# Hi-PACE/hipace

Measured on AMD Instinct MI355X. Metric: transverse slices/s at 1024^2 x 4ppc (explicit solver), higher is better.
Workload: dtype f64

## Files before the change

hipace_amd/csrc/particles_tiled.hip:

```cpp
#include "common.h"
#include <type_traits>
#include "particle_math.h"
#include "tiling.h"
#include "mg_gate.h"
#include "beam_deposit.h"

#include <algorithm>
#include <atomic>
#include <cstdio>
#include <cstdlib>
#include <cstring>
#include <mutex>
#include <set>
#include <string>

namespace hps {

static std::atomic<bool> g_record{false};
static std::mutex g_record_mu;
static std::set<std::string> g_recorded;
static void record_launch (const char* kernel, std::initializer_list<int> args)
{
    std::string n(kernel);
    char sep = '<';
    for (int a : args) { char b[16]; std::snprintf(b, sizeof b, "%c%d", sep, a); n += b; sep = ','; }
    n += '>';
    std::lock_guard<std::mutex> lk(g_record_mu);
    g_recorded.insert(n);
}
#define HPS_RECORD(kernel, ...) do { if (__builtin_expect(g_record.load(std::memory_order_relaxed), 0)) record_launch(kernel, {__VA_ARGS__}); } while (0)

static int expl_pad ()
{
    static int pad = -1;
    if (pad < 0) {
        pad = 2;
        if (const char* e = std::getenv("HPS_EXPL_PAD")) { const int v = std::atoi(e); if (v == 2 || v == 8) pad = v; }
    }
    return pad;
}
constexpr int TILE_HALO = 6;

#ifdef HPS_STAMPS
__device__ long long* g_pt_dbg = nullptr;
#define PT_STAMP(i) do { if (g_pt_dbg && blockIdx.x == 2000 && threadIdx.x == 0) g_pt_dbg[i] = __builtin_amdgcn_s_memtime(); } while (0)
#else
#define PT_STAMP(i) do { } while (0)
#endif

struct CompSlots { int n; int comp[6]; };

typedef __attribute__((address_space(3))) double lds_double;

__device__ __forceinline__ void lds_add (double* p, double v)
{
    __hip_atomic_fetch_add((lds_double*)p, v, __ATOMIC_RELAXED, __HIP_MEMORY_SCOPE_WORKGROUP);
}
__device__ __forceinline__ double lds_get (const double* p)
{
    return *(const lds_double*)p;
}

template <int ORDER>
__device__ __forceinline__ double laser_gather_lds (const double* a, int pitch, int li, int lj, const double* lx, const double* ly)
{
    double A = 0.0;
#pragma unroll
    for (int iy = 0; iy <= ORDER; ++iy)
#pragma unroll
        for (int ix = 0; ix <= ORDER; ++ix) A += lx[ix]*ly[iy]*lds_get(a + (lj + iy)*pitch + li + ix);
    return A;
}
template <int ORDER>
__device__ __forceinline__ void laser_gather_grad_lds (const double* a, int pitch, int li, int lj, const double* lx, const double* ly,
                                                       double dx_inv, double dy_inv, double& A, double& ADx, double& ADy)
{
    A = 0.0; ADx = 0.0; ADy = 0.0;
#pragma unroll
    for (int iy = 0; iy <= ORDER; ++iy)
#pragma unroll
        for (int ix = 0; ix <= ORDER; ++ix) {
            const double* c = a + (lj + iy)*pitch + li + ix;
            const double w = lx[ix]*ly[iy];
            A += w*lds_get(c);
            ADx += w*0.5*dx_inv*(lds_get(c + 1) - lds_get(c - 1));
            ADy += w*0.5*dy_inv*(lds_get(c + pitch) - lds_get(c - pitch));
        }
}

__device__ __forceinline__ int4 tile_record (const int* __restrict__ offsets, const TailWork& tw, long n, bool& tail)
{
    const int b0 = (int)blockIdx.x - tw.extra;
    const int b = b0 - tw.nwg;
    tail = b < 0;
    if (tail) {
        const long nn = tw.live_n ? (long)*tw.live_n : n;
        const long first = (long)tw.first + 256L*b0;
        return make_int4(0, (int)min(first, nn), (int)min(first + 256, nn), 0);
    }
    return reinterpret_cast<const int4*>(offsets + tile_launch_offset(gridDim.x - tw.nwg - tw.extra))[b];
}
constexpr int TAIL_ORIGIN = -(1 << 24);

template <int R, int RP = R, int NT = 256, int NC = 6>
__device__ __forceinline__ void load_region (double* img, const SlabView& f, const int* comps, int nc, int ox, int oy, int tid);

template <int ORDER, int TS, int MASK, bool LASER = false, bool VBW = false>
__global__ __launch_bounds__(256)
void k_deposit_tiled (SlabView f, hps_plasma pl, const int* __restrict__ offsets, int ntx, DepComps cm,
                      PartConsts k, int* n_qsa, int* n_fallback, const int* __restrict__ tile_flag, TailWork tw, BeamPairWork bw,
                      const int* go)
{
    if (go && *go == 0) return;
    if ((int)blockIdx.x < bw.nwg) {
        beam_pair_block<ORDER>(f, bw, (int)blockIdx.x, k.dx_inv, k.dy_inv, k.xoff, k.yoff);
        return;
    }
    constexpr int R = TS + 2*TILE_HALO;
    constexpr int RP = R, PL = RP*R;
    if (tile_flag && !tile_flag[offsets[gridDim.x + 2 + blockIdx.x]]) return;
    extern __shared__ __attribute__((aligned(16))) double acc[];
    const int gc[6] = {cm.jx, cm.jy, cm.jz, cm.rho, cm.chi, cm.rhomjz};
    int slot[6]; int na = 0;
#pragma unroll
    for (int c = 0; c < 6; ++c) {
        const bool on = (MASK >= 0) ? ((MASK >> c) & 1) : (gc[c] >= 0);
        slot[c] = on ? na++ : -1;
    }

    bool tail;
    const int4 lrec = tile_record(offsets, tw, pl.n, tail);
    const int tile = lrec.x;
    const int ox = tail ? TAIL_ORIGIN : (tile % ntx)*TS - TILE_HALO, oy = tail ? TAIL_ORIGIN : (tile / ntx)*TS - TILE_HALO;
    const int tid = threadIdx.x;
    PT_STAMP(0);
    const int pend = lrec.z;
    int nfb = 0;
    struct Rec { double x, y, w, ux, uy, psi; uint64_t id; int ion; };
    auto fetch = [&] (int ip) {
        Rec r;
        r.x = pl.x[ip]; r.y = pl.y[ip]; r.w = pl.w[ip];
        r.ux = pl.ux[ip]; r.uy = pl.uy[ip]; r.psi = pl.psi[ip];
        if constexpr (VBW) r.id = (r.w != 0.0) ? HPS_ID_VALID : 0ULL;
        else r.id = pl.idcpu[ip];
        r.ion = k.can_ionize ? pl.ion_lev[ip] : 1;
        return r;
    };
    constexpr int NB = 4;
    Rec rec[NB];
    const int ipb = lrec.y + tid;
    if (ipb < pend) {
#pragma unroll
        for (int u = 0; u < NB; ++u) rec[u] = fetch(min(ipb + 256*u, pend - 1));
    }
    {
        double2* z = (double2*)acc;
        for (int s = tid; s < na*PL/2; s += 256) z[s] = make_double2(0.0, 0.0);
    }
    double* aimg = acc + na*PL;
    if constexpr (LASER) { const int ca[1] = {k.aabs}; load_region<R, R, 256, 1>(aimg, f, ca, 1, ox, oy, tid); }
    __syncthreads();
    PT_STAMP(1);

    for (int ip0 = ipb; ip0 < pend; ip0 += 256*NB) {
      if (ip0 != ipb) {
#pragma unroll
        for (int u = 0; u < NB; ++u) rec[u] = fetch(min(ip0 + 256*u, pend - 1));
      }
#pragma unroll
      for (int u = 0; u < NB; ++u) {
        const int ip = ip0 + 256*u;
        if (ip >= pend) break;
        const Rec cur = rec[u];
        const uint64_t id = cur.id;
        if (!(id & HPS_ID_VALID)) continue;
        const double psi_inv = 1.0/cur.psi;
        const double vx_c = cur.ux*psi_inv;
        const double vy_c = cur.uy*psi_inv;
        double q_invvol = k.a*cur.w;
        double q_mu0_mass = k.b;
        if (k.can_ionize) { const double il = (double)cur.ion; q_invvol *= il; q_mu0_mass *= il; }
        double sx[ORDER + 1], sy[ORDER + 1];
        const int i0 = shape_weights<ORDER>((cur.x - k.xoff)*k.dx_inv, sx);
        const int j0 = shape_weights<ORDER>((cur.y - k.yoff)*k.dy_inv, sy);
        const int li = i0 - ox, lj = j0 - oy;
        const bool local = (li >= 0 && li + ORDER < R && lj >= 0 && lj + ORDER < R);
        double gamma_psi;
        if constexpr (LASER) {
            double A = (local ? laser_gather_lds<ORDER>(aimg, R, li, lj, sx, sy)
                              : laser_gather<ORDER>(f, k.aabs, (cur.x - k.xoff)*k.dx_inv, (cur.y - k.yoff)*k.dy_inv))*k.laser_fac;
            if (k.can_ionize) A *= (double)cur.ion*(double)cur.ion;
            gamma_psi = 0.5*((1.0 + 0.5*A)*psi_inv*psi_inv + vx_c*vx_c*k.c_inv*k.c_inv + vy_c*vy_c*k.c_inv*k.c_inv + 1.0);
        } else {
            gamma_psi = 0.5*(psi_inv*psi_inv + vx_c*vx_c*k.c_inv*k.c_inv + vy_c*vy_c*k.c_inv*k.c_inv + 1.0);
        }
        if (gamma_psi < 0.0 || gamma_psi > k.max_qsa || psi_inv < 0.0) {
            if (n_qsa) atomicAdd(n_qsa, 1);
            pl.w[ip] = 0.0;
            pl.idcpu[ip] = (VBW ? pl.idcpu[ip] : id) & ~HPS_ID_VALID;
            if (pl.psi_half) pl.psi_half[ip] = 0.0;
            continue;
        }
        if (k.can_ionize && cur.ion == 0) continue;
        const double wv[6] = {vx_c, vy_c, (gamma_psi - 1.0)*k.c, gamma_psi, q_mu0_mass*psi_inv, 1.0};
        if (local) {
#pragma unroll
            for (int iy = 0; iy <= ORDER; ++iy) {
#pragma unroll
                for (int ix = 0; ix <= ORDER; ++ix) {
                    const double cd = q_invvol*sx[ix]*sy[iy];
                    double* p = acc + (lj + iy)*RP + li + ix;
#pragma unroll
                    for (int c = 0; c < 6; ++c) if (slot[c] >= 0) lds_add(p + slot[c]*PL, cd*wv[c]);
                }
            }
        } else {
            nfb += !tail;
#pragma unroll
            for (int iy = 0; iy <= ORDER; ++iy) {
#pragma unroll
                for (int ix = 0; ix <= ORDER; ++ix) {
                    const double cd = q_invvol*sx[ix]*sy[iy];
                    double* p = f.p + f.off(i0 + ix, j0 + iy);
#pragma unroll
                    for (int c = 0; c < 6; ++c) if (slot[c] >= 0) atomic_add_f64(p + gc[c]*f.ns, cd*wv[c]);
                }
            }
        }
      }
    }
    if (n_fallback && nfb) atomicAdd(n_fallback, nfb);
    PT_STAMP(2);
    __syncthreads();
    PT_STAMP(3);

    for (int s = tid; s < R*R; s += 256) {
        const int lj = s / R, li = s - lj*R;
        const int i = ox + li, j = oy + lj;
        if (i < -f.ng || i >= f.nx + f.ng || j < -f.ng || j >= f.ny + f.ng) continue;
        double* p = f.p + f.off(i, j);
#pragma unroll
        for (int c = 0; c < 6; ++c) {
            if (slot[c] >= 0) {
                const double v = acc[slot[c]*PL + lj*RP + li];
                if (v != 0.0) atomic_add_f64(p + gc[c]*f.ns, v);
            }
        }
    }
    PT_STAMP(4);
}

template <int R, int RP, int NT, int NC>
__device__ __forceinline__ void load_region (double* img, const SlabView& f, const int* comps, int nc, int ox, int oy, int tid)
{
    constexpr int NIT = (R*R + NT - 1)/NT;
    double v[NIT][NC];
#pragma unroll
    for (int it = 0; it < NIT; ++it) {
        const int s = min(tid + it*NT, R*R - 1);
        const int lj = s / R, li = s - lj*R;
        const int i = ox + li, j = oy + lj;
        const bool in = (i >= -f.ng && i < f.nx + f.ng && j >= -f.ng && j < f.ny + f.ng);
        const long o = in ? f.off(i, j) : 0;
#pragma unroll
        for (int c = 0; c < NC; ++c) { v[it][c] = 0.0; if (c < nc) { const double q = f.p[comps[c]*f.ns + o]; v[it][c] = in ? q : 0.0; } }
    }
#pragma unroll
    for (int it = 0; it < NIT; ++it) {
        const int s = tid + it*NT;
        if (s < R*R) {
            const int lj = s / R, li = s - lj*R;
#pragma unroll
            for (int c = 0; c < NC; ++c) if (c < nc) img[c*RP*R + lj*RP + li] = v[it][c];
        }
    }
}

template <int ORDER, int DT, int TS, bool LASER = false, int PAD = 2, bool VBW = false>
__global__ __launch_bounds__(256) __attribute__((amdgpu_waves_per_eu(4, 4)))
void k_explicit_tiled (SlabView f, hps_plasma pl, const int* __restrict__ offsets, int ntx,
                       int cBz, int cEz, int cExmBy, int cEypBx, int cSy, int cSx, PartConsts k, int* n_fallback,
                       const int* __restrict__ tile_flag, TailWork tw)
{
    constexpr int R = TS + 2*TILE_HALO;
    constexpr int RP = R + PAD, PL = RP*R;
    if (tile_flag && !tile_flag[offsets[gridDim.x + 2 + blockIdx.x]]) return;
    constexpr int NS = ORDER + DT + 1;
    extern __shared__ __attribute__((aligned(16))) double lds[];
    double* img = lds;
    double* acc = lds + 4*PL;
    double* aimg = lds + 6*PL;
    bool tail;
    const int4 lrec = tile_record(offsets, tw, pl.n, tail);
    const int tile = lrec.x;
    const int ox = tail ? TAIL_ORIGIN : (tile % ntx)*TS - TILE_HALO, oy = tail ? TAIL_ORIGIN : (tile / ntx)*TS - TILE_HALO;
    const int tid = threadIdx.x;
    const int cc[4] = {cBz, cEz, cExmBy, cEypBx};
    const int pend = lrec.z;
    struct Rec { double x, y, w, ux, uy, psi; uint64_t id; int ion; };
    auto fetch = [&] (int ip) {
        Rec r;
        r.x = pl.x[ip]; r.y = pl.y[ip]; r.w = pl.w[ip];
        r.ux = pl.ux[ip]; r.uy = pl.uy[ip]; r.psi = pl.psi[ip];
        if constexpr (VBW) r.id = (r.w != 0.0) ? HPS_ID_VALID : 0ULL;
        else r.id = pl.idcpu[ip];
        r.ion = k.can_ionize ? pl.ion_lev[ip] : 1;
        return r;
    };
    const int ipb = lrec.y + tid;
    Rec nxt{};
    if (ipb < pend) nxt = fetch(ipb);
    load_region<R, RP, 256, 4>(img, f, cc, 4, ox, oy, tid);
    if constexpr (LASER) { const int ca[1] = {k.aabs}; load_region<R, RP, 256, 1>(aimg, f, ca, 1, ox, oy, tid); }
    {
        double2* z = (double2*)acc;
        for (int s = tid; s < PL; s += 256) z[s] = make_double2(0.0, 0.0);
    }
    __syncthreads();

    int nfb = 0;
    bool slow = false;
    auto one = [&] (const Rec& cur, auto LC) __attribute__((always_inline)) -> bool {
        constexpr bool LOCAL = decltype(LC)::value;
        if (!(cur.id & HPS_ID_VALID)) return true;
        if (k.can_ionize && cur.ion == 0) return true;
        const double xmid = (cur.x - k.xoff)*k.dx_inv;
        const double ymid = (cur.y - k.yoff)*k.dy_inv;
        double sx[NS], dsx[NS], sy[NS], dsy[NS];
        int i0, j0;
        if constexpr (DT == 2) { i0 = centred_weights<ORDER>(xmid, sx, dsx); j0 = centred_weights<ORDER>(ymid, sy, dsy); }
        else                   { i0 = nodal_weights<ORDER>(xmid, sx, dsx);   j0 = nodal_weights<ORDER>(ymid, sy, dsy); }
        const int li = i0 - ox, lj = j0 - oy;
        const bool local = LASER ? (li >= 1 && li + NS + 1 <= R && lj >= 1 && lj + NS + 1 <= R)
                                 : (li >= 0 && li + NS <= R && lj >= 0 && lj + NS <= R);
        if (local != LOCAL) return false;
        const double psi_inv = fast_rcp(cur.psi);
        const double vx = cur.ux*psi_inv*k.c_inv;
        const double vy = cur.uy*psi_inv*k.c_inv;
        double q_invvol_mu0 = k.a, q_mass = k.b;
        if (k.can_ionize) { const double il = (double)cur.ion; q_invvol_mu0 *= il; q_mass *= il; }
        const double cdm = q_invvol_mu0*cur.w;
        double gp;
        if constexpr (LASER) {
            double lx[ORDER + 1], ly[ORDER + 1];
            const int ai = shape_weights<ORDER>(xmid, lx), aj = shape_weights<ORDER>(ymid, ly);
            const double A = (LOCAL ? laser_gather_lds<ORDER>(aimg, RP, ai - ox, aj - oy, lx, ly)
                                    : laser_gather<ORDER>(f, k.aabs, xmid, ymid))*k.laser_fac*q_mass*q_mass;
            gp = 0.5*((1.0 + 0.5*A)*psi_inv*psi_inv + vx*vx + vy*vy + 1.0);
        } else {
            gp = 0.5*(psi_inv*psi_inv + vx*vx + vy*vy + 1.0);
        }
        const double qp = q_mass*psi_inv;
        const double vxvy = vx*vy, gy = gp - vy*vy, gx = gp - vx*vx;
        const double cq = cdm*qp, cqc = cq*k.c_inv, cc = cdm*k.c;
        const double a1 = cq*vx, a2 = -cqc*vy, a3 = cqc*vxvy, a4 = -cqc*gy, a5 = cc*vxvy, a6 = -cc*(gy - 1.0);
        const double b1 = cq*vy, b2 = cqc*vx, b3 = cqc*gx, b4 = -cqc*vxvy, b5 = cc*(gx - 1.0), b6 = -cc*vxvy;
#pragma unroll
        for (int m = 0; m < NS; ++m) { dsx[m] *= k.dx_inv; dsy[m] *= k.dy_inv; }
#pragma unroll
        for (int iy = 0; iy < NS; ++iy) {
            if constexpr (LOCAL) asm volatile("" ::: "memory");
            const bool yedge = (DT == 2) && (iy == 0 || iy == NS - 1);
            const double a5s = a5*sy[iy], b5s = b5*sy[iy], ay = a6*dsy[iy], by = b6*dsy[iy];
#pragma unroll
            for (int ix = 0; ix < NS; ++ix) {
                const bool xedge = (DT == 2) && (ix == 0 || ix == NS - 1);
                if (xedge && yedge) continue;
                double* gp_ = nullptr; int ls = 0;
                if constexpr (LOCAL) ls = (lj + iy)*RP + li + ix;
                else                 gp_ = f.p + f.off(i0 + ix, j0 + iy);
                double sy_add, sx_add;
                if (xedge)      { sy_add = a5s*dsx[ix]; sx_add = b5s*dsx[ix]; }
                else if (yedge) { sy_add = ay*sx[ix];   sx_add = by*sx[ix]; }
                else {
                    double Bz, Ez, ExmBy, EypBx;
                    if constexpr (LOCAL) { Bz = lds_get(img + ls); Ez = lds_get(img + PL + ls); ExmBy = lds_get(img + 2*PL + ls); EypBx = lds_get(img + 3*PL + ls); }
                    else                 { Bz = gp_[cBz*f.ns]; Ez = gp_[cEz*f.ns]; ExmBy = gp_[cExmBy*f.ns]; EypBx = gp_[cEypBx*f.ns]; }
                    double ty = fma(a1, Bz, fma(a2, Ez, fma(a3, ExmBy, a4*EypBx)));
                    double tx = fma(b1, Bz, fma(b2, Ez, fma(b3, ExmBy, b4*EypBx)));
                    if constexpr (LASER) {
                        if (sx[ix]*sy[iy] != 0.0) {
                            const double lf = 0.25*cq*qp*k.laser_fac*k.c;
                            double ady, adx;
                            if constexpr (LOCAL) {
                                const double* a = aimg + ls;
                                ady = lds_get(a + RP) - lds_get(a - RP); adx = lds_get(a + 1) - lds_get(a - 1);
                            } else {
                                const double* a = f.p + k.aabs*f.ns + f.off(i0 + ix, j0 + iy);
                                ady = a[f.js] - a[-f.js]; adx = a[1] - a[-1];
                            }
                            ty = fma(lf*0.5*k.dy_inv, ady, ty);
                            tx = fma(-lf*0.5*k.dx_inv, adx, tx);
                        }
                    }
                    sy_add = fma(sx[ix], fma(sy[iy], ty, ay), a5s*dsx[ix]);
                    sx_add = fma(sx[ix], fma(sy[iy], tx, by), b5s*dsx[ix]);
                }
                if constexpr (LOCAL) { lds_add(acc + ls, sy_add); lds_add(acc + PL + ls, sx_add); }
                else                 { atomic_add_f64(gp_ + cSy*f.ns, sy_add); atomic_add_f64(gp_ + cSx*f.ns, sx_add); }
            }
        }
        return true;
    };
    for (int ip = ipb; ip < pend; ip += 256) {
        const Rec cur = nxt;
        if (ip + 256 < pend) nxt = fetch(ip + 256);
        if (!one(cur, std::true_type{})) { slow = true; nfb += !tail; }
    }
    if (slow) {
#pragma unroll 1
        for (int ip = ipb; ip < pend; ip += 256) { const Rec cur = fetch(ip); (void)one(cur, std::false_type{}); }
    }
    if (n_fallback && nfb) atomicAdd(n_fallback, nfb);
    __syncthreads();
#ifdef HPS_DIAG_EXPL_NO_FLUSH
    if (acc[tid] == 1.2345e-300 && n_fallback) atomicAdd(n_fallback, 1);
    return;
#endif
    for (int s = tid; s < R*R; s += 256) {
        const int lj = s / R, li = s - lj*R;
        const int i = ox + li, j = oy + lj;
        if (i < -f.ng || i >= f.nx + f.ng || j < -f.ng || j >= f.ny + f.ng) continue;
        double* p = f.p + f.off(i, j);
        const double a = acc[lj*RP + li], b = acc[PL + lj*RP + li];
        if (a != 0.0) atomic_add_f64(p + cSy*f.ns, a);
        if (b != 0.0) atomic_add_f64(p + cSx*f.ns, b);
    }
}

template <class T> __device__ __forceinline__ T ldo (const T* base, unsigned o) { return *reinterpret_cast<const T*>(reinterpret_cast<const char*>(base) + o); }
template <class T> __device__ __forceinline__ void sto (T* base, unsigned o, T v) { *reinterpret_cast<T*>(reinterpret_cast<char*>(base) + o) = v; }
template <class T> __device__ __forceinline__ T ldo_nt (const T* base, unsigned o) { return __builtin_nontemporal_load(reinterpret_cast<const T*>(reinterpret_cast<const char*>(base) + o)); }
template <class T> __device__ __forceinline__ void sto_nt (T* base, unsigned o, T v) { __builtin_nontemporal_store(v, reinterpret_cast<T*>(reinterpret_cast<char*>(base) + o)); }

struct DepTail { DepComps cm; double a, b, max_qsa; int* n_qsa; };
template <int ORDER, int TS, bool LASER = false, bool IONIZE = false, bool VBP = false, int DEP = 0>
__global__ __launch_bounds__(256) __attribute__((amdgpu_waves_per_eu(IONIZE ? 2 : 3)))
void k_advance_tiled (SlabView f, hps_plasma pl, const int* __restrict__ offsets, int ntx,
                      int cPsi, int cEz, int cBx, int cBy, int cBz, PartConsts k, int* n_fallback, IonArgs ia, const int* go, TailWork tw, MgPost mp,
                      DepTail dt)
{
    static_assert(DEP == 0 || (!LASER && !IONIZE), "the deposition tail exists for the plain push only");
    constexpr int R = TS + 2*TILE_HALO;
    constexpr int NS = ORDER + 2;
    static_assert(!(VBP && IONIZE), "the ADK draw is keyed by the id");
    int go_now;
    if (mp.src) {
        go_now = vcycle_active(mp.after) ? 0 : 1;
        if (blockIdx.x == 0) {
            for (int w = threadIdx.x; w < mp.nwords; w += 256) mp.dst[w] = mp.src[w];
            HPS_HOST_STORES_ACKNOWLEDGED();
            __syncthreads();
            if (threadIdx.x == 0) *mp.seq_slot = mp.seq;
        }
    } else go_now = go ? *go : 1;
    int charged = 0;
    extern __shared__ __attribute__((aligned(16))) double img[];
    bool tail;
    const int4 lrec = tile_record(offsets, tw, pl.n, tail);
    const int tile = lrec.x;
    if constexpr (IONIZE) {
        if (!go_now) return;
        if (ia.fbound && ia.tile_flag && ia.tile_flag[tile] == 0 && adk_tile_below_threshold(ia, tile % ntx, tile / ntx)) {
            adk_post(ia);
            return;
        }
    }
    const int ox = tail ? TAIL_ORIGIN : (tile % ntx)*TS - TILE_HALO, oy = tail ? TAIL_ORIGIN : (tile / ntx)*TS - TILE_HALO;
    const int tid = threadIdx.x;
    const unsigned pend = (unsigned)lrec.z;
    struct PIn { uint64_t id; double xp, yp, uxh, uyh, psih; };
    auto fetch = [&] (unsigned ip) {
        PIn q;
        const unsigned o = ip*8u;
        if constexpr (!VBP) q.id = ldo(pl.idcpu, o);
        q.xp = ldo(pl.x_prev, o); q.yp = ldo(pl.y_prev, o);
        q.uxh = ldo_nt(pl.ux_half, o); q.uyh = ldo_nt(pl.uy_half, o); q.psih = ldo_nt(pl.psi_half, o);
        if constexpr (VBP) q.id = (q.psih != 0.0) ? HPS_ID_VALID : 0ULL;
        return q;
    };
    unsigned ip = (unsigned)lrec.y + tid;
    PIn nxt{0, 0.0, 0.0, 0.0, 0.0, 1.0};
    if (ip < pend) nxt = fetch(ip);
    const int cc[5] = {cPsi, cEz, cBx, cBy, cBz};
    load_region<R, R, 256, 5>(img, f, cc, 5, ox, oy, tid);
    double* aimg = img + 5*R*R;
    if constexpr (LASER) { const int ca[1] = {k.aabs}; load_region<R, R, 256, 1>(aimg, f, ca, 1, ox, oy, tid); }
    __syncthreads();
    if (!go_now) return;
    int nfb = 0;

    for (; ip < pend; ip += 256) {
        __builtin_assume(ip < (1u << 28));
        const PIn cur = nxt;
        if (ip + 256 < pend) nxt = fetch(ip + 256);
        const unsigned o8 = ip*8u;
        const uint64_t id = cur.id;
        if (!(id & HPS_ID_VALID)) continue;
        double qmc = k.a;
        if (k.can_ionize) qmc *= (double)pl.ion_lev[ip];
        bool dead = false;
        for (int isc = 0; isc < k.n_subcycles && !dead; ++isc) {
            double xp = isc == 0 ? cur.xp : ldo(pl.x_prev, o8);
            double yp = isc == 0 ? cur.yp : ldo(pl.y_prev, o8);
            double sx[NS], dsx[NS], sy[NS], dsy[NS];
            constexpr bool W3 = ORDER == 2;
            double pxw[3] = {0.0, 0.0, 0.0}, pyw[3] = {0.0, 0.0, 0.0}; bool xhw = false, yhw = false;
            int i0, j0;
            if constexpr (W3) {
                i0 = nodal_weights2_w3((xp - k.xoff)*k.dx_inv, sx, dsx, pxw, xhw);
                j0 = nodal_weights2_w3((yp - k.yoff)*k.dy_inv, sy, dsy, pyw, yhw);
            } else {
                i0 = nodal_weights<ORDER>((xp - k.xoff)*k.dx_inv, sx, dsx);
                j0 = nodal_weights<ORDER>((yp - k.yoff)*k.dy_inv, sy, dsy);
            }
            const int li = i0 - ox, lj = j0 - oy;
            const bool local = (li >= 0 && li + NS <= R && lj >= 0 && lj + NS <= R);
            if (!local && !tail) ++nfb;
            Fld F{0, 0, 0, 0, 0, 0};
            if (local) {
                const double* b = img + lj*R + li;
#pragma unroll
                for (int iy = 0; iy < NS; ++iy) {
                    double rp = 0.0, rd = 0.0;
#pragma unroll
                    for (int ix = 0; ix < NS; ++ix) {
                        const double psi_c = lds_get(b + iy*R + ix);
                        rp = fma(sx[ix], psi_c, rp);
                        rd = fma(dsx[ix], psi_c, rd);
                    }
                    F.ExmBy = fma(sy[iy], rd, F.ExmBy);
                    F.EypBx = fma(dsy[iy], rp, F.EypBx);
                }
                const bool xhi = W3 ? xhw : !(sx[NS - 1] == 0.0), yhi = W3 ? yhw : !(sy[NS - 1] == 0.0);
                double px[NS - 1], py[NS - 1];
#pragma unroll
                for (int m = 0; m < NS - 1; ++m) {
                    if constexpr (W3) { px[m] = pxw[m < 3 ? m : 2]; py[m] = pyw[m < 3 ? m : 2]; }
                    else { px[m] = xhi ? sx[m + 1] : sx[m]; py[m] = yhi ? sy[m + 1] : sy[m]; }
                }
                const double* bq = b + R*R + (yhi ? R : 0) + (xhi ? 1 : 0);
#pragma unroll
                for (int ky = 0; ky < NS - 1; ++ky) {
                    asm volatile("" ::: "memory");
                    double rez = 0.0, rbx = 0.0, rby = 0.0, rbz = 0.0;
#pragma unroll
                    for (int kx = 0; kx < NS - 1; ++kx) {
                        const int ls = ky*R + kx;
                        rez = fma(px[kx], lds_get(bq + ls), rez);
                        rbx = fma(px[kx], lds_get(bq + R*R + ls), rbx);
                        rby = fma(px[kx], lds_get(bq + 2*R*R + ls), rby);
                        rbz = fma(px[kx], lds_get(bq + 3*R*R + ls), rbz);
                    }
                    F.Ez  = fma(py[ky], rez, F.Ez);
                    F.Bxc = fma(py[ky], rbx, F.Bxc);
                    F.Byc = fma(py[ky], rby, F.Byc);
                    F.Bz  = fma(py[ky], rbz, F.Bz);
                }
                F.ExmBy *= k.dx_inv;
                F.EypBx *= k.dy_inv;
            } else {
#ifdef HPS_DIAG_PUSH_NO_FALLBACK
                F.Ez = 1.0;
#else
#pragma unroll 1
                for (int iy = 0; iy < NS; ++iy) {
#pragma unroll
                    for (int ix = 0; ix < NS; ++ix) {
                        const double* p = f.p + f.off(i0 + ix, j0 + iy);
                        const double psi_c = p[cPsi*f.ns];
                        const double ss = sx[ix]*sy[iy];
                        F.ExmBy += (dsx[ix]*sy[iy])*psi_c*k.dx_inv;
                        F.EypBx += (sx[ix]*dsy[iy])*psi_c*k.dy_inv;
                        F.Ez  += ss*p[cEz*f.ns];
                        F.Bxc += ss*p[cBx*f.ns];
                        F.Byc += ss*p[cBy*f.ns];
                        F.Bz  += ss*p[cBz*f.ns];
                    }
                }
#endif
            }
            F.Bxc *= k.c;
            F.Byc *= k.c;
            if constexpr (IONIZE) {
                if (isc == 0) {
                    int lev = pl.ion_lev[ip];
                    const double uxh = cur.uxh, uyh = cur.uyh;
                    const bool ionize = lev < ia.Z && adk_decide(ia, F.ExmBy + F.Byc, F.EypBx - F.Bxc, F.Ez, uxh, uyh, cur.psih, lev, id);
                    if (ionize) { ++lev; pl.ion_lev[ip] = lev; qmc = k.a*(double)lev; }
                    adk_emit(ia, ionize, pl.x[ip], pl.y[ip], xp, yp, pl.w[ip]);
                    charged |= (lev > 0);
                    if (lev == 0 && uxh == 0.0 && uyh == 0.0) break;
                }
            }
            LaserFld Lf{0.0, 0.0, 0.0};
            if constexpr (LASER) {
                double lx[ORDER + 1], ly[ORDER + 1];
                const int ai = shape_weights<ORDER>((xp - k.xoff)*k.dx_inv, lx) - ox, aj = shape_weights<ORDER>((yp - k.yoff)*k.dy_inv, ly) - oy;
                if (ai >= 1 && ai + ORDER + 1 < R && aj >= 1 && aj + ORDER + 1 < R)
                    laser_gather_grad_lds<ORDER>(aimg, R, ai, aj, lx, ly, k.dx_inv, k.dy_inv, Lf.A, Lf.ADx, Lf.ADy);
                else
                    laser_gather_grad<ORDER>(f, k.aabs, (xp - k.xoff)*k.dx_inv, (yp - k.yoff)*k.dy_inv, k.dx_inv, k.dy_inv, Lf.A, Lf.ADx, Lf.ADy);
                const double ln = k.laser_fac*(k.can_ionize ? (double)pl.ion_lev[ip]*(double)pl.ion_lev[ip] : 1.0);
                Lf.A *= 0.5*ln; Lf.ADx *= 0.25*k.c*ln; Lf.ADy *= 0.25*k.c*ln;
            }
            const double dz = k.dz, sdz = dz*0.25;
            double ux = isc == 0 ? cur.uxh : ldo(pl.ux_half, o8), uy = isc == 0 ? cur.uyh : ldo(pl.uy_half, o8), psi = isc == 0 ? cur.psih : ldo(pl.psi_half, o8);
            const PushForce PFc = push_force(F, Lf, k.c_inv, qmc);
            const double h2 = 0.5*sdz*sdz;
#pragma unroll 1
            for (int s = 0; s < 4; ++s) taylor2_substep_pre<LASER>(ux, uy, psi, PFc, sdz, h2);
            const double pinv = fast_rcp(psi);
            xp += dz*k.c_inv*(ux*pinv);
            yp += dz*k.c_inv*(uy*pinv);
            if (apply_particle_bc(k, xp, yp, ux, uy)) {
                sto(pl.w, o8, 0.0);
                sto(pl.idcpu, o8, (uint64_t)((VBP ? ldo(pl.idcpu, o8) : id) & ~HPS_ID_VALID));
                sto(pl.psi_half, o8, 0.0);
                dead = true;
                break;
            }
            sto(pl.x, o8, xp); sto(pl.y, o8, yp);
            if (!k.temp_slice) {
                sto_nt(pl.ux_half, o8, ux); sto_nt(pl.uy_half, o8, uy); sto_nt(pl.psi_half, o8, psi);
                if (pl.x_prev != pl.x) sto(pl.x_prev, o8, xp);
                if (pl.y_prev != pl.y) sto(pl.y_prev, o8, yp);
            }
#pragma unroll 1
            for (int s = 0; s < 2; ++s) taylor2_substep_pre<LASER>(ux, uy, psi, PFc, sdz, h2);
            sto(pl.ux, o8, ux); sto(pl.uy, o8, uy); sto(pl.psi, o8, psi);
        }
    }
    if constexpr (DEP != 0) {
        constexpr int RR = R*R;
        const int gc[6] = {dt.cm.jx, dt.cm.jy, dt.cm.jz, dt.cm.rho, dt.cm.chi, dt.cm.rhomjz};
        int slot[6]; int na = 0;
#pragma unroll
        for (int c = 0; c < 6; ++c) { const bool on = (DEP >> c) & 1; slot[c] = on ? na++ : -1; }
        __syncthreads();
        double* acc = img;
        {   double2* z = (double2*)acc;
            for (int s2 = tid; s2 < na*RR/2; s2 += 256) z[s2] = make_double2(0.0, 0.0); }
        __syncthreads();
        for (unsigned iq = (unsigned)lrec.y + tid; iq < pend; iq += 256) {
            const unsigned o = iq*8u;
            auto ldc2 = [] (const double* base, unsigned off) {
                return __hip_atomic_load(reinterpret_cast<const double*>(reinterpret_cast<const char*>(base) + off), __ATOMIC_RELAXED, __HIP_MEMORY_SCOPE_AGENT); };
            const double w = ldc2(pl.w, o);
            const double x = ldc2(pl.x, o), y = ldc2(pl.y, o), ux = ldc2(pl.ux, o), uy = ldc2(pl.uy, o), psi = ldc2(pl.psi, o);
            if (w == 0.0) continue;
            const double psi_inv = 1.0/psi;
            const double vx_c = ux*psi_inv, vy_c = uy*psi_inv;
            const double q_invvol = dt.a*w;
            const double gamma_psi = 0.5*(psi_inv*psi_inv + vx_c*vx_c*k.c_inv*k.c_inv + vy_c*vy_c*k.c_inv*k.c_inv + 1.0);
            if (gamma_psi < 0.0 || gamma_psi > dt.max_qsa || psi_inv < 0.0) {
                if (dt.n_qsa) atomicAdd(dt.n_qsa, 1);
                sto(pl.w, o, 0.0);
                sto(pl.idcpu, o, (uint64_t)(ldo(pl.idcpu, o) & ~HPS_ID_VALID));
                sto(pl.psi_half, o, 0.0);
                continue;
            }
            double wx[ORDER + 1], wy[ORDER + 1];
            const int i0 = shape_weights<ORDER>((x - k.xoff)*k.dx_inv, wx);
            const int j0 = shape_weights<ORDER>((y - k.yoff)*k.dy_inv, wy);
            const double wv[6] = {vx_c, vy_c, (gamma_psi - 1.0)*k.c, gamma_psi, dt.b*psi_inv, 1.0};
            const int li = i0 - ox, lj = j0 - oy;
            if (li >= 0 && li + ORDER < R && lj >= 0 && lj + ORDER < R) {
#pragma unroll
                for (int iy = 0; iy <= ORDER; ++iy) {
#pragma unroll
                    for (int ix = 0; ix <= ORDER; ++ix) {
                        const double cd = q_invvol*wx[ix]*wy[iy];
                        double* p = acc + (lj + iy)*R + li + ix;
#pragma unroll
                        for (int c = 0; c < 6; ++c) if (slot[c] >= 0) lds_add(p + slot[c]*RR, cd*wv[c]);
                    }
                }
            } else {
                nfb += !tail;
#pragma unroll
                for (int iy = 0; iy <= ORDER; ++iy) {
#pragma unroll
                    for (int ix = 0; ix <= ORDER; ++ix) {
                        const double cd = q_invvol*wx[ix]*wy[iy];
                        double* p = f.p + f.off(i0 + ix, j0 + iy);
#pragma unroll
                        for (int c = 0; c < 6; ++c) if (slot[c] >= 0) atomic_add_f64(p + gc[c]*f.ns, cd*wv[c]);
                    }
                }
            }
        }
        __syncthreads();
        for (int s2 = tid; s2 < RR; s2 += 256) {
            const int lj = s2 / R, li = s2 - lj*R;
            const int i = ox + li, j = oy + lj;
            if (i < -f.ng || i >= f.nx + f.ng || j < -f.ng || j >= f.ny + f.ng) continue;
            double* p = f.p + f.off(i, j);
#pragma unroll
            for (int c = 0; c < 6; ++c) {
                if (slot[c] >= 0) {
                    const double v = acc[slot[c]*RR + s2];
                    if (v != 0.0) atomic_add_f64(p + gc[c]*f.ns, v);
                }
            }
        }
    }
    if (n_fallback && nfb) atomicAdd(n_fallback, nfb);
    if constexpr (IONIZE) {
        const int any = __syncthreads_or(charged);
        if (ia.tile_flag && tid == 0) ia.tile_flag[tile] = any;
        adk_post(ia);
    }
}

template <int ORDER, int TS, int MASK, int NT>
__global__ __launch_bounds__(NT)
void k_advance_deposit_tiled (SlabView f, hps_plasma pl, const int* __restrict__ offsets, int ntx,
                              int cPsi, int cEz, int cBx, int cBy, int cBz, PartConsts k, DepComps cm, PartConsts kd,
                              int* n_qsa, int* n_fallback)
{
    constexpr int R = TS + 2*TILE_HALO;
    constexpr int NS = ORDER + 2;
    extern __shared__ __attribute__((aligned(16))) double img[];
    double* acc = img + 5*R*R;
    const int gc[6] = {cm.jx, cm.jy, cm.jz, cm.rho, cm.chi, cm.rhomjz};
    int slot[6]; int na = 0;
#pragma unroll
    for (int c = 0; c < 6; ++c) { const bool on = (MASK >> c) & 1; slot[c] = on ? na++ : -1; }
    const int tile = offsets[gridDim.x + 2 + blockIdx.x];
    const int ox = (tile % ntx)*TS - TILE_HALO, oy = (tile / ntx)*TS - TILE_HALO;
    const int tid = threadIdx.x;
    const int cc[5] = {cPsi, cEz, cBx, cBy, cBz};
    load_region<R, R, NT, 5>(img, f, cc, 5, ox, oy, tid);
    {
        double2* z = (double2*)acc;
        for (int s = tid; s < na*R*R/2; s += NT) z[s] = make_double2(0.0, 0.0);
    }
    __syncthreads();

    const int pend = offsets[tile + 1];
    int nfb = 0;
    for (int ip = offsets[tile] + tid; ip < pend; ip += NT) {
        const uint64_t id = pl.idcpu[ip];
        if (!(id & HPS_ID_VALID)) continue;
        const double qmc = k.a;
        bool dead = false;
        double xp = 0.0, yp = 0.0, ux = 0.0, uy = 0.0, psi = 1.0;
        for (int isc = 0; isc < k.n_subcycles && !dead; ++isc) {
            xp = pl.x_prev[ip];
            yp = pl.y_prev[ip];
            double sx[NS], dsx[NS], sy[NS], dsy[NS];
            const int i0 = nodal_weights<ORDER>((xp - k.xoff)*k.dx_inv, sx, dsx);
            const int j0 = nodal_weights<ORDER>((yp - k.yoff)*k.dy_inv, sy, dsy);
            const int li = i0 - ox, lj = j0 - oy;
            const bool local = (li >= 0 && li + NS <= R && lj >= 0 && lj + NS <= R);
            if (!local) ++nfb;
            Fld F{0, 0, 0, 0, 0, 0};
            if (local) {
                const double* b = img + lj*R + li;
#pragma unroll 1
                for (int iy = 0; iy < NS; ++iy) {
                    double rp = 0.0, rd = 0.0, rez = 0.0, rbx = 0.0, rby = 0.0, rbz = 0.0;
#pragma unroll
                    for (int ix = 0; ix < NS; ++ix) {
                        const int ls = iy*R + ix;
                        const double psi_c = lds_get(b + ls);
                        rp = fma(sx[ix], psi_c, rp);
                        rd = fma(dsx[ix], psi_c, rd);
                        rez = fma(sx[ix], lds_get(b + R*R + ls), rez);
                        rbx = fma(sx[ix], lds_get(b + 2*R*R + ls), rbx);
                        rby = fma(sx[ix], lds_get(b + 3*R*R + ls), rby);
                        rbz = fma(sx[ix], lds_get(b + 4*R*R + ls), rbz);
                    }
                    F.ExmBy = fma(sy[iy], rd, F.ExmBy);
                    F.EypBx = fma(dsy[iy], rp, F.EypBx);
                    F.Ez  = fma(sy[iy], rez, F.Ez);
                    F.Bxc = fma(sy[iy], rbx, F.Bxc);
                    F.Byc = fma(sy[iy], rby, F.Byc);
                    F.Bz  = fma(sy[iy], rbz, F.Bz);
                }
                F.ExmBy *= k.dx_inv;
                F.EypBx *= k.dy_inv;
            } else {
#pragma unroll 1
                for (int iy = 0; iy < NS; ++iy) {
#pragma unroll
                    for (int ix = 0; ix < NS; ++ix) {
                        const double* p = f.p + f.off(i0 + ix, j0 + iy);
                        const double psi_c = p[cPsi*f.ns];
                        const double ss = sx[ix]*sy[iy];
                        F.ExmBy += (dsx[ix]*sy[iy])*psi_c*k.dx_inv;
                        F.EypBx += (sx[ix]*dsy[iy])*psi_c*k.dy_inv;
                        F.Ez  += ss*p[cEz*f.ns];
                        F.Bxc += ss*p[cBx*f.ns];
                        F.Byc += ss*p[cBy*f.ns];
                        F.Bz  += ss*p[cBz*f.ns];
                    }
                }
            }
            F.Bxc *= k.c;
            F.Byc *= k.c;
            const double dz = k.dz, sdz = dz*0.25;
            ux = pl.ux_half[ip]; uy = pl.uy_half[ip]; psi = pl.psi_half[ip];
#pragma unroll 1
            for (int s = 0; s < 4; ++s) taylor2_substep(ux, uy, psi, F, k.c_inv, qmc, sdz);
            const double pinv = fast_rcp(psi);
            xp += dz*k.c_inv*(ux*pinv);
            yp += dz*k.c_inv*(uy*pinv);
            if (apply_particle_bc(k, xp, yp, ux, uy)) {
                pl.w[ip] = 0.0;
                pl.idcpu[ip] = id & ~HPS_ID_VALID;
                pl.psi_half[ip] = 0.0;
                dead = true;
                break;
            }
            pl.x[ip] = xp; pl.y[ip] = yp;
            pl.ux_half[ip] = ux; pl.uy_half[ip] = uy; pl.psi_half[ip] = psi;
            if (pl.x_prev != pl.x) pl.x_prev[ip] = xp;
            if (pl.y_prev != pl.y) pl.y_prev[ip] = yp;
#pragma unroll 1
            for (int s = 0; s < 2; ++s) taylor2_substep(ux, uy, psi, F, k.c_inv, qmc, sdz);
            pl.ux[ip] = ux; pl.uy[ip] = uy; pl.psi[ip] = psi;
        }
        if (dead) continue;
        const double w = pl.w[ip];
        const double psi_inv = 1.0/psi;
        const double vx_c = ux*psi_inv;
        const double vy_c = uy*psi_inv;
        const double q_invvol = kd.a*w;
        const double gamma_psi = 0.5*(psi_inv*psi_inv + vx_c*vx_c*kd.c_inv*kd.c_inv + vy_c*vy_c*kd.c_inv*kd.c_inv + 1.0);
        if (gamma_psi < 0.0 || gamma_psi > kd.max_qsa || psi_inv < 0.0) {
            if (n_qsa) atomicAdd(n_qsa, 1);
            pl.w[ip] = 0.0;
            pl.idcpu[ip] = id & ~HPS_ID_VALID;
            pl.psi_half[ip] = 0.0;
            continue;
        }
        double wx[ORDER + 1], wy[ORDER + 1];
        const int i0 = shape_weights<ORDER>((xp - kd.xoff)*kd.dx_inv, wx);
        const int j0 = shape_weights<ORDER>((yp - kd.yoff)*kd.dy_inv, wy);
        const double wv[6] = {vx_c, vy_c, (gamma_psi - 1.0)*kd.c, gamma_psi, kd.b*psi_inv, 1.0};
        const int li = i0 - ox, lj = j0 - oy;
        if (li >= 0 && li + ORDER < R && lj >= 0 && lj + ORDER < R) {
#pragma unroll
            for (int iy = 0; iy <= ORDER; ++iy) {
#pragma unroll
                for (int ix = 0; ix <= ORDER; ++ix) {
                    const double cd = q_invvol*wx[ix]*wy[iy];
                    double* p = acc + (lj + iy)*R + li + ix;
#pragma unroll
                    for (int c = 0; c < 6; ++c) if (slot[c] >= 0) lds_add(p + slot[c]*R*R, cd*wv[c]);
                }
            }
        } else {
            ++nfb;
#pragma unroll
            for (int iy = 0; iy <= ORDER; ++iy) {
#pragma unroll
                for (int ix = 0; ix <= ORDER; ++ix) {
                    const double cd = q_invvol*wx[ix]*wy[iy];
                    double* p = f.p + f.off(i0 + ix, j0 + iy);
#pragma unroll
                    for (int c = 0; c < 6; ++c) if (slot[c] >= 0) atomic_add_f64(p + gc[c]*f.ns, cd*wv[c]);
                }
            }
        }
    }
    if (n_fallback && nfb) atomicAdd(n_fallback, nfb);
    __syncthreads();
    for (int s = tid; s < R*R; s += NT) {
        const int lj = s / R, li = s - lj*R;
        const int i = ox + li, j = oy + lj;
        if (i < -f.ng || i >= f.nx + f.ng || j < -f.ng || j >= f.ny + f.ng) continue;
        double* p = f.p + f.off(i, j);
#pragma unroll
        for (int c = 0; c < 6; ++c) {
            if (slot[c] >= 0) {
                const double v = acc[slot[c]*R*R + s];
                if (v != 0.0) atomic_add_f64(p + gc[c]*f.ns, v);
            }
        }
    }
}

template <class K>
static int set_lds (K kernel, size_t bytes)
{
    if (bytes > 64*1024) HPS_HIP_CHECK(hipFuncSetAttribute((const void*)kernel, hipFuncAttributeMaxDynamicSharedMemorySize, (int)bytes));
    return HPS_OK;
}

#define HPS_DISPATCH_ORDER_TS(order, ts, CALL)                                   \
    switch ((order)*100 + (ts)) {                                                \
        case   16: { CALL(0, 16); } break;  case   32: { CALL(0, 32); } break;    \
        case  116: { CALL(1, 16); } break;  case  132: { CALL(1, 32); } break;    \
        case  216: { CALL(2, 16); } break;  case  232: { CALL(2, 32); } break;    \
        case  316: { CALL(3, 16); } break;  case  332: { CALL(3, 32); } break;    \
        default: set_error("tiled kernels: unsupported order / tile size"); return HPS_ERR_ARG; }

int deposit_current_tiled (const hps_slab& slab, const hps_plasma& pl, const hps_geom& g, const int comp[6], double charge,
                           double mass, int order, double max_qsa, int can_ionize, int* n_qsa, Tiling* T, int* n_fallback,
                           hipStream_t st, int aabs_comp, const int* tile_flag, TailWork tw, const BeamPairWork* beam, const int* go,
                           bool valid_by_w)
{
    if (pl.n == 0) return HPS_OK;
    const BeamPairWork bw = beam ? *beam : BeamPairWork{};
    tw.extra = bw.nwg;
    HPS_REQUIRE(!(tile_flag && (tw.nwg || bw.nwg)), "deposit_current_tiled: tile flags cannot be combined with tail or beam workgroups");
    HPS_REQUIRE(pl.n + 256L*tw.nwg < (1L << 28), "deposit_current_tiled: the tile kernels address at most 2^28 particles per sheet");
    PartConsts k = base_consts(g);
    k.a = charge*invvol_of(g); k.b = charge*g.mu0/mass; k.max_qsa = max_qsa; k.can_ionize = can_ionize;
    k.aabs = aabs_comp; k.laser_fac = (charge/g.q_e)*(g.m_e/mass)*(charge/g.q_e)*(g.m_e/mass);
    DepComps cm{comp[0], comp[1], comp[2], comp[3], comp[4], comp[5]};
    int na = 0; for (int c = 0; c < 6; ++c) na += comp[c] >= 0;
    {   int m = 0; for (int c = 0; c < 6; ++c) m |= (comp[c] >= 0) << c;
        k.valid_by_w = valid_by_w && !tw.nwg && aabs_comp < 0 && (m == 51 || m == 3); }
    const int R = T->g.ts + 2*TILE_HALO;
    const size_t lds = ((size_t)na*R*R + (aabs_comp >= 0 ? (size_t)R*R : 0))*sizeof(double);
    SlabView f(slab);
    int mask = 0; for (int c = 0; c < 6; ++c) mask |= (comp[c] >= 0) << c;
#define CALLM(O, S, M) { if (int e = set_lds(k_deposit_tiled<O, S, M>, lds)) return e; HPS_RECORD("k_deposit_tiled", O, S, M, 0, 0); \
        hipLaunchKernelGGL((k_deposit_tiled<O, S, M>), dim3(T->g.ntiles + tw.nwg + bw.nwg), dim3(256), lds, st, f, pl, T->offsets, T->g.ntx, cm, k, n_qsa, n_fallback, tile_flag, tw, bw, go); }
#define CALLL(O, S, M) { if (int e = set_lds(k_deposit_tiled<O, S, M, true>, lds)) return e; HPS_RECORD("k_deposit_tiled", O, S, M, 1, 0); \
        hipLaunchKernelGGL((k_deposit_tiled<O, S, M, true>), dim3(T->g.ntiles + tw.nwg + bw.nwg), dim3(256), lds, st, f, pl, T->offsets, T->g.ntx, cm, k, n_qsa, n_fallback, tile_flag, tw, bw, go); }
#define CALLV(O, S, M) { if (int e = set_lds(k_deposit_tiled<O, S, M, false, true>, lds)) return e; HPS_RECORD("k_deposit_tiled", O, S, M, 0, 1); \
        hipLaunchKernelGGL((k_deposit_tiled<O, S, M, false, true>), dim3(T->g.ntiles + tw.nwg + bw.nwg), dim3(256), lds, st, f, pl, T->offsets, T->g.ntx, cm, k, n_qsa, n_fallback, tile_flag, tw, bw, go); }
#define CALL(O, S) { if (aabs_comp >= 0) { if (mask == 51) CALLL(O, S, 51) else CALLL(O, S, -1) } \
                     else if (k.valid_by_w && mask == 51) CALLV(O, S, 51) else if (k.valid_by_w && mask == 3) CALLV(O, S, 3) \
                     else if (mask == 51) CALLM(O, S, 51) else if (mask == 59) CALLM(O, S, 59) else if (mask == 32) CALLM(O, S, 32) \
                     else if (mask == 3) CALLM(O, S, 3) else if (mask == 39) CALLM(O, S, 39) else if (mask == 47) CALLM(O, S, 47) else CALLM(O, S, -1) }
    HPS_DISPATCH_ORDER_TS(order, T->g.ts, CALL)
#undef CALL
#undef CALLM
#undef CALLL
// ... 247 lines not shown
```

Measured before the change: 1668.

## Defer particle push stores and fence prefetch loads to overlap memory with compute

Restructures the particle push loop so each particle's results are returned in a struct and committed after the next particle's prefetch is issued, with asm barriers keeping the prefetched registers live. Adds explicit s_waitcnt vmcnt(0) fences before the main loops and between subcycles. Moves the validity check (w or psi nonzero) from the fetch into the processing step, so the prefetch no longer waits on the loaded value. The aim is to let outstanding global loads and stores overlap with compute instead of serialising on waitcnt, at the cost of more live registers and a risk of lower occupancy.

Measured after the change: 1715 (median of 6 runs). +2.8%, better.

```diff
diff --git a/hipace_amd/csrc/particles_tiled.hip b/hipace_amd/csrc/particles_tiled.hip
--- a/hipace_amd/csrc/particles_tiled.hip
+++ b/hipace_amd/csrc/particles_tiled.hip
@@ -60,6 +60,8 @@
 {
     return *(const lds_double*)p;
 }
+
+__device__ __forceinline__ void vm_wait_all () { __builtin_amdgcn_s_waitcnt(0x0F70); }
 
 template <int ORDER>
 __device__ __forceinline__ double laser_gather_lds (const double* a, int pitch, int li, int lj, const double* lx, const double* ly)
@@ -302,7 +304,7 @@
         Rec r;
         r.x = pl.x[ip]; r.y = pl.y[ip]; r.w = pl.w[ip];
         r.ux = pl.ux[ip]; r.uy = pl.uy[ip]; r.psi = pl.psi[ip];
-        if constexpr (VBW) r.id = (r.w != 0.0) ? HPS_ID_VALID : 0ULL;
+        if constexpr (VBW) r.id = 0ULL;
         else r.id = pl.idcpu[ip];
         r.ion = k.can_ionize ? pl.ion_lev[ip] : 1;
         return r;
@@ -322,7 +324,7 @@
     bool slow = false;
     auto one = [&] (const Rec& cur, auto LC) __attribute__((always_inline)) -> bool {
         constexpr bool LOCAL = decltype(LC)::value;
-        if (!(cur.id & HPS_ID_VALID)) return true;
+        if (VBW ? !(cur.w != 0.0) : !(cur.id & HPS_ID_VALID)) return true;
         if (k.can_ionize && cur.ion == 0) return true;
         const double xmid = (cur.x - k.xoff)*k.dx_inv;
         const double ymid = (cur.y - k.yoff)*k.dy_inv;
@@ -402,6 +404,7 @@
         }
         return true;
     };
+    vm_wait_all();
     for (int ip = ipb; ip < pend; ip += 256) {
         const Rec cur = nxt;
         if (ip + 256 < pend) nxt = fetch(ip + 256);
@@ -476,7 +479,7 @@
         if constexpr (!VBP) q.id = ldo(pl.idcpu, o);
         q.xp = ldo(pl.x_prev, o); q.yp = ldo(pl.y_prev, o);
         q.uxh = ldo_nt(pl.ux_half, o); q.uyh = ldo_nt(pl.uy_half, o); q.psih = ldo_nt(pl.psi_half, o);
-        if constexpr (VBP) q.id = (q.psih != 0.0) ? HPS_ID_VALID : 0ULL;
+        if constexpr (VBP) q.id = 0ULL;
         return q;
     };
     unsigned ip = (unsigned)lrec.y + tid;
@@ -490,19 +493,33 @@
     if (!go_now) return;
     int nfb = 0;
 
-    for (; ip < pend; ip += 256) {
-        __builtin_assume(ip < (1u << 28));
-        const PIn cur = nxt;
-        if (ip + 256 < pend) nxt = fetch(ip + 256);
+    struct POut { int kind; uint64_t id; double xp, yp, uxh, uyh, psih, ux, uy, psi; };
+    auto commit = [&] (const POut& r, unsigned o8) __attribute__((always_inline)) {
+        asm volatile("" : "+v"(o8));
+        if (r.kind == 1) {
+            sto(pl.w, o8, 0.0);
+            sto(pl.idcpu, o8, (uint64_t)((VBP ? ldo(pl.idcpu, o8) : r.id) & ~HPS_ID_VALID));
+            sto(pl.psi_half, o8, 0.0);
+        } else if (r.kind == 2) {
+            sto(pl.x, o8, r.xp); sto(pl.y, o8, r.yp);
+            if (!k.temp_slice) {
+                sto_nt(pl.ux_half, o8, r.uxh); sto_nt(pl.uy_half, o8, r.uyh); sto_nt(pl.psi_half, o8, r.psih);
+                if (pl.x_prev != pl.x) sto(pl.x_prev, o8, r.xp);
+                if (pl.y_prev != pl.y) sto(pl.y_prev, o8, r.yp);
+            }
+            sto(pl.ux, o8, r.ux); sto(pl.uy, o8, r.uy); sto(pl.psi, o8, r.psi);
+        }
+    };
+    auto process = [&] (const PIn& cur, unsigned ip) __attribute__((always_inline)) -> POut {
+        POut r{};
         const unsigned o8 = ip*8u;
-        const uint64_t id = cur.id;
-        if (!(id & HPS_ID_VALID)) continue;
+        const uint64_t id = VBP ? ((cur.psih != 0.0) ? HPS_ID_VALID : 0ULL) : cur.id;
+        r.id = id;
+        if (!(id & HPS_ID_VALID)) return r;
         double qmc = k.a;
         if (k.can_ionize) qmc *= (double)pl.ion_lev[ip];
-        bool dead = false;
-        for (int isc = 0; isc < k.n_subcycles && !dead; ++isc) {
-            double xp = isc == 0 ? cur.xp : ldo(pl.x_prev, o8);
-            double yp = isc == 0 ? cur.yp : ldo(pl.y_prev, o8);
+        double xp = cur.xp, yp = cur.yp, ux = cur.uxh, uy = cur.uyh, psi = cur.psih;
+        for (int isc = 0; isc < k.n_subcycles; ++isc) {
             double sx[NS], dsx[NS], sy[NS], dsy[NS];
             constexpr bool W3 = ORDER == 2;
             double pxw[3] = {0.0, 0.0, 0.0}, pyw[3] = {0.0, 0.0, 0.0}; bool xhw = false, yhw = false;
@@ -590,7 +607,7 @@
                     if (ionize) { ++lev; pl.ion_lev[ip] = lev; qmc = k.a*(double)lev; }
                     adk_emit(ia, ionize, pl.x[ip], pl.y[ip], xp, yp, pl.w[ip]);
                     charged |= (lev > 0);
-                    if (lev == 0 && uxh == 0.0 && uyh == 0.0) break;
+                    if (lev == 0 && uxh == 0.0 && uyh == 0.0) return r;
                 }
             }
             LaserFld Lf{0.0, 0.0, 0.0};
@@ -605,7 +622,6 @@
                 Lf.A *= 0.5*ln; Lf.ADx *= 0.25*k.c*ln; Lf.ADy *= 0.25*k.c*ln;
             }
             const double dz = k.dz, sdz = dz*0.25;
-            double ux = isc == 0 ? cur.uxh : ldo(pl.ux_half, o8), uy = isc == 0 ? cur.uyh : ldo(pl.uy_half, o8), psi = isc == 0 ? cur.psih : ldo(pl.psi_half, o8);
             const PushForce PFc = push_force(F, Lf, k.c_inv, qmc);
             const double h2 = 0.5*sdz*sdz;
 #pragma unroll 1
@@ -613,23 +629,32 @@
             const double pinv = fast_rcp(psi);
             xp += dz*k.c_inv*(ux*pinv);
             yp += dz*k.c_inv*(uy*pinv);
-            if (apply_particle_bc(k, xp, yp, ux, uy)) {
-                sto(pl.w, o8, 0.0);
-                sto(pl.idcpu, o8, (uint64_t)((VBP ? ldo(pl.idcpu, o8) : id) & ~HPS_ID_VALID));
-                sto(pl.psi_half, o8, 0.0);
-                dead = true;
-                break;
-            }
-            sto(pl.x, o8, xp); sto(pl.y, o8, yp);
-            if (!k.temp_slice) {
-                sto_nt(pl.ux_half, o8, ux); sto_nt(pl.uy_half, o8, uy); sto_nt(pl.psi_half, o8, psi);
-                if (pl.x_prev != pl.x) sto(pl.x_prev, o8, xp);
-                if (pl.y_prev != pl.y) sto(pl.y_prev, o8, yp);
-            }
+            if (apply_particle_bc(k, xp, yp, ux, uy)) { r.kind = 1; return r; }
+            r.xp = xp; r.yp = yp; r.uxh = ux; r.uyh = uy; r.psih = psi;
 #pragma unroll 1
             for (int s = 0; s < 2; ++s) taylor2_substep_pre<LASER>(ux, uy, psi, PFc, sdz, h2);
-            sto(pl.ux, o8, ux); sto(pl.uy, o8, uy); sto(pl.psi, o8, psi);
-        }
+            r.ux = ux; r.uy = uy; r.psi = psi;
+            r.kind = 2;
+            if (isc + 1 < k.n_subcycles) {
+                commit(r, o8);
+                r.kind = 0;
+                unsigned o = o8;
+                asm volatile("" : "+v"(o));
+                xp = ldo(pl.x_prev, o); yp = ldo(pl.y_prev, o);
+                ux = ldo(pl.ux_half, o); uy = ldo(pl.uy_half, o); psi = ldo(pl.psi_half, o);
+                vm_wait_all();
+            }
+        }
+        return r;
+    };
+    vm_wait_all();
+    for (; ip < pend; ip += 256) {
+        __builtin_assume(ip < (1u << 28));
+        const PIn cur = nxt;
+        if (ip + 256 < pend) nxt = fetch(ip + 256);
+        const POut r = process(cur, ip);
+        asm volatile("" : "+v"(nxt.id), "+v"(nxt.xp), "+v"(nxt.yp), "+v"(nxt.uxh), "+v"(nxt.uyh), "+v"(nxt.psih) :: "memory");
+        commit(r, ip*8u);
     }
     if constexpr (DEP != 0) {
         constexpr int RR = R*R;
```
